# 2noise/ChatTTS

Measured on AMD Instinct MI355X. Metric: audio seconds/sec (RTF), batch=64 per GPU, higher is better.
Workload: dtype f32x3

## Files before the change

### chattts_amd/_lib.py

```python
from __future__ import annotations

import ctypes as C
import os

import numpy as np

import torch

HERE = os.path.dirname(os.path.abspath(__file__))
LIB_PATH = os.environ.get("CTTS_LIB") or os.path.join(HERE, "csrc", "libchattts_amd.so")

F32, BF16 = 0, 1
P = C.c_void_p
PP = C.POINTER(C.c_void_p)


class GptWeights(C.Structure):
    _fields_ = [
        ("n_layers", C.c_int32), ("weight_dtype", C.c_int32), ("kv_dtype", C.c_int32), ("max_pos", C.c_int32),
        ("wqkv", PP), ("wo", PP), ("wgu", PP), ("wd", PP), ("ln1", PP), ("ln2", PP),
        ("norm", P), ("emb_code", P), ("heads", P), ("rope_cos", P), ("rope_sin", P),
        ("rms_eps", C.c_float),
        ("emb_text", P), ("head_text", P), ("n_text", C.c_int32),
        ("wqkv_pk", PP), ("wo_pk", PP), ("wgu_pk", PP), ("wd_pk", PP),
# ... 84 lines not shown
        ("encoder", TrunkWeights), ("decoder", TrunkWeights),
        ("ds0_w", P), ("ds0_b", P), ("ds1_w", P), ("ds1_b", P), ("out_conv_w", P), ("coef", P),
        ("q_in_w", P), ("q_in_b", P), ("q_out_w", P), ("q_out_b", P),
        ("levels", C.c_int32 * 4), ("G", C.c_int32), ("R", C.c_int32), ("D", C.c_int32), ("bound_first", C.c_int32),
        ("mel_window", P), ("mel_fb", P), ("twiddle", P),
    ]


I32, F, SZ = C.c_int32, C.c_float, C.c_size_t

SIGNATURES = {
    "ctts_last_error": (C.c_char_p, []),
    "ctts_version": (C.c_int, []),
    "ctts_gpt_create": (C.c_int, [PP, C.POINTER(GptWeights)]),
    "ctts_gpt_destroy": (None, [P]),
    "ctts_gpt_workspace_bytes": (SZ, [I32, I32]),
    "ctts_gpt_prefill": (C.c_int, [P, C.POINTER(GenState), P, P]),
    "ctts_gpt_prefill_chunk": (C.c_int, [P, C.POINTER(GenState), P, I32, I32, I32, P]),
    "ctts_gpt_decode_step": (C.c_int, [P, C.POINTER(GenState), P]),
    "ctts_gpt_graph_build": (C.c_int, [P, C.POINTER(GenState), P]),
    "ctts_gpt_graph_launch": (C.c_int, [P, I32, P]),
    "ctts_gpt_graph_build_rows": (C.c_int, [P, C.POINTER(GenState), I32, P]),
    "ctts_gpt_graph_launch_rows": (C.c_int, [P, I32, I32, P]),
    "ctts_gpt_graph_destroy": (None, [P]),
    "ctts_gpt_profile_begin": (C.c_int, [P, I32, I32, I32]),
    "ctts_gpt_profile_samples": (C.c_int, [P, C.POINTER(C.c_float), I32, C.POINTER(I32)]),
    "ctts_gpt_profile_end": (C.c_int, [P, C.POINTER(I32), C.POINTER(C.c_double)]),
    "ctts_codec_create": (C.c_int, [PP, C.POINTER(CodecWeights)]),
    "ctts_codec_destroy": (None, [P]),
    "ctts_codec_workspace_bytes": (SZ, [I32, I32]),
# ... 35 lines not shown
    "ctts_dvae_encode_workspace_bytes": (SZ, [I32]),
    "ctts_dvae_decode_workspace_bytes": (SZ, [I32, I32]),
    "ctts_dvae_encode": (C.c_int, [P, P, I32, P, P, SZ, P]),
    "ctts_dvae_decode_codes": (C.c_int, [P, P, P, I32, I32, P, SZ, P]),
    "ctts_k_gemm": (C.c_int, [I32, P, P, P, I32, I32, I32, I32, I32, I32, I32, P, F, P, I32, P, P, I32, I32, I32, I32, I32, P]),
    "ctts_k_gemm_x3p": (C.c_int, [P, P, I32, I32, I32, I32, P, P, P, P, P, P]),
    "ctts_k_gemm_h1p": (C.c_int, [P, P, I32, I32, I32, I32, P, P, P, P, P, P]),
    "ctts_stream_create_cu_mask": (C.c_int, [I32, I32, I32, I32, P]),
    "ctts_stream_destroy": (C.c_int, [P]),
    "ctts_k_mlp_fused": (C.c_int, [P, P, P, I32, I32, P, P, P, P, I32, P]),
    "ctts_k_gemm_fast": (C.c_int, [P, I32, P, I32, I32, I32, P, F, I32, P, I32, P, I32, P, P]),
    "ctts_k_qkv_rope": (C.c_int, [P, P, I32, P, F, P, P, P, I32, P, P, I32, P, P, I32, P]),
    "ctts_k_gemm_dec": (C.c_int, [P, P, I32, I32, I32, P, P, F, I32, P, I32, P, I32, P, I32, P]),
    "ctts_k_gemm_dec32x": (C.c_int, [P, C.c_int64, P, C.c_int64, I32, I32, I32, P, P, I32, F, I32, P, I32, P, I32, P, C.c_int64, I32, P, I32, P, P, P]),
    "ctts_k_gemm_pre_x3": (C.c_int, [P, I32, P, P, I32, I32, I32, I32, I32, P, P, P, I32, P]),
    "ctts_k_dec32_last_variant": (C.c_char_p, []),
    "ctts_k_gemm_dec32": (C.c_int, [P, P, I32, I32, I32, P, P, I32, P, F, I32, P, I32, P, I32, P, I32, I32, I32, P]),
    "ctts_k_rows_prep": (C.c_int, [P, P, P, I32, P]),
    "ctts_k_rope_append": (C.c_int, [P, P, P, I32, I32, P, P, I32, P, P, I32, P]),
    "ctts_k_attention": (C.c_int, [P, P, P, I32, I32, P, I32, P, P, I32, P]),
    "ctts_k_attention_prefill": (C.c_int, [P, P, P, I32, P, I32, I32, P, I32, P]),
    "ctts_k_attention_dec": (C.c_int, [P, P, P, I32, P, P, P, I32, P, P, I32, P]),
    "ctts_k_attention_dec2": (C.c_int, [P, P, P, I32, I32, P, P, P, I32, I32, P]),
    "ctts_k_attention_cfg": (C.c_int, [I32, I32, I32]),
    "ctts_k_attention_heads_per_wg": (C.c_int, [I32]),
    "ctts_rccl_unique_id": (C.c_int, [P]),
    "ctts_rccl_comm_create": (C.c_int, [P, I32, P, I32]),
    "ctts_rccl_comm_destroy": (None, [P]),
    "ctts_broadcast_weights": (C.c_int, [P, P, I32, P, I32, P]),
    "ctts_k_attention_oproj": (C.c_int, [P, P, P, I32, P, P, P, I32, P, P, P, P, P, P]),
# ... 57 lines not shown
```

### chattts_amd/csrc/capi.hip

```cpp
#include <hip/hip_runtime.h>
#include <dlfcn.h>
#include <stdarg.h>
#include <stdio.h>
#include <stdlib.h>
#include <string.h>
#include <algorithm>
#include <map>
#include <vector>

#include "../../include/chattts_amd.h"
#include "kernels.hpp"

static thread_local char g_err[512] = "";
int ctts_fail(const char* fmt, ...) {
  va_list ap;
  va_start(ap, fmt);
  vsnprintf(g_err, sizeof(g_err), fmt, ap);
  va_end(ap);
  return -1;
}
#define fail ctts_fail
#define CK(expr)                                                                                   \
  do {                                                                                             \
    hipError_t _e = (expr);                                                                        \
// ... 11 lines not shown
  std::vector<const void*> wqkv_pk, wo_pk, wgu_pk, wd_pk;
  std::vector<const void*> wo_hd;
  std::vector<const void*> wqkv_x3, wo_x3, wgu_x3, wd_x3;
  bool dec_x3 = false;
  bool qkv_att = false;
  bool att_oproj = false;
  bool dec_packed = false;
  bool dec_packed32 = false;
  bool heads_packed = false;
  int pf_mask = 0;
  int temporal_layers = 0;
  bool pre32_packed = true;
  bool embed_fold = false;
  bool pre_compact = true;
  bool pre_x3 = true;
  bool fnorm_fuse = true;
  std::vector<const float*> ln1, ln2;
  hipGraph_t graph = nullptr;
  hipGraphExec_t exec = nullptr;
  hipGraph_t graph_multi = nullptr;
  hipGraphExec_t exec_multi = nullptr;
  struct RowsGraph { hipGraph_t graph = nullptr, gm = nullptr; hipGraphExec_t exec = nullptr, exec_multi = nullptr; };
  std::map<int, RowsGraph> rows_graphs;
  int multi_steps = 1;
  int prof_tag = -1;
  int prof_max = 0;
  bool skip_finished = true;
  int n_cu = 0;
  int prof_stride = 1;
  int prof_seen = 0;
// ... 92 lines not shown
    g->dec_x3 = true;
  }
  if (w->wo_hd && g->dec_packed) {
    g->wo_hd.assign(w->wo_hd, w->wo_hd + L);
    const char* e = getenv("CTTS_ATT_OPROJ");
    g->att_oproj = e && atoi(e) == 1;
  }
  { const char* e = getenv("CTTS_SKIP_FINISHED"); if (e && atoi(e) == 0) g->skip_finished = false; }
  { const char* e = getenv("CTTS_FNORM_FUSE"); if (e && atoi(e) == 0) g->fnorm_fuse = false; }
  { const char* e = getenv("CTTS_W_TEMPORAL_LAYERS"); if (e) g->temporal_layers = atoi(e); }
  { const char* e = getenv("CTTS_PF"); if (e) g->pf_mask = atoi(e); }
  { const char* e = getenv("CTTS_QKV_ATT"); g->qkv_att = e && atoi(e) == 1; }
  { const char* e = getenv("CTTS_PRE32_PACKED"); if (e && atoi(e) == 0) g->pre32_packed = false; }
  { const char* e = getenv("CTTS_PRE_X3"); if (e && atoi(e) == 0) g->pre_x3 = false; }
  { const char* e = getenv("CTTS_PRE_COMPACT"); if (e && atoi(e) == 0) g->pre_compact = false; }
  { const char* e = getenv("CTTS_EMBED_FOLD"); if (e) g->embed_fold = atoi(e) != 0; }
  {
    int dev = 0, cus = 0;
    const char* e = getenv("CTTS_ATT_SPLIT");
    if (e && atoi(e) == 1 && hipGetDevice(&dev) == hipSuccess &&
        hipDeviceGetAttribute(&cus, hipDeviceAttributeMultiprocessorCount, dev) == hipSuccess && cus > 0 && cus <= ATT_CUS_MAX)
      g->n_cu = cus;
  }
  *out = g;
  return 0;
}

extern "C" void ctts_gpt_graph_destroy(ctts_gpt* g) {
  if (!g) return;
  if (g->exec) { (void)hipGraphExecDestroy(g->exec); g->exec = nullptr; }
  if (g->graph) { (void)hipGraphDestroy(g->graph); g->graph = nullptr; }
  if (g->exec_multi) { (void)hipGraphExecDestroy(g->exec_multi); g->exec_multi = nullptr; }
  if (g->graph_multi) { (void)hipGraphDestroy(g->graph_multi); g->graph_multi = nullptr; }
  for (auto& kv : g->rows_graphs) {
    if (kv.second.exec) (void)hipGraphExecDestroy(kv.second.exec);
    if (kv.second.graph) (void)hipGraphDestroy(kv.second.graph);
    if (kv.second.exec_multi) (void)hipGraphExecDestroy(kv.second.exec_multi);
    if (kv.second.gm) (void)hipGraphDestroy(kv.second.gm);
  }
// ... 254 lines not shown
    d.res = nullptr; d.Cp = ws.actp32; d.kch_out = INTER / 16;
    CK(launch_gemm_pre32(d, ws.rstd, st));
    d.Ap = ws.actp32; d.Wp = (const float*)g->wd_pk[l]; d.N = HID; d.K = INTER; d.norm_w = nullptr; d.epi = EPI_RES;
    d.C = ws.x; d.ldc = HID; d.res = ws.x; d.ldr = HID; d.Cp = ws.xp32; d.kch_out = HID / 16;
    CK(launch_gemm_pre32(d, nullptr, st));
  }
  for (int l = 0; !fast && !packed32 && !pre32 && !x3 && l < g->w.n_layers; ++l) {
    void* kc = (char*)s->kcache + kv_layer * l;
    void* vc = (char*)s->vcache + kv_layer * l;
    GemmArgs a;
    memset(&a, 0, sizeof(a));
    a.taps = 1;
    a.n_active = nact;
    a.A = ws.x; a.lda = HID; a.W = g->wqkv[l]; a.C = ws.qkv; a.ldc = 3 * HID; a.M = M; a.N = 3 * HID; a.K = HID; a.wt = wt;
    a.epi = EPI_STORE; a.norm_w = g->ln1[l]; a.eps = g->w.rms_eps;
    if (pre_x3) { CK(launch_rows_rstd32(ws.x, HID, M, g->w.rms_eps, ws.rstd, st)); CK(launch_gemm_pre_x3(a, ws.rstd, st)); }
    else { Prof p(g, 1, st, prof_ok); CK(launch_gemm_skinny(a, st)); }
    { Prof p(g, 2, st, prof_ok); CK(launch_rope_append(ws.qkv, kc, vc, kt, cmax, g->w.rope_cos, g->w.rope_sin, rm, M, st)); }
    { Prof p(g, 3, st, prof_ok); CK(launch_attention(ws.qkv, kc, vc, kt, cmax, ws.ao, 0, rm, M, st)); }
    a.A = ws.ao; a.lda = HID; a.W = g->wo[l]; a.C = ws.x; a.ldc = HID; a.N = HID; a.K = HID; a.epi = EPI_RES; a.norm_w = nullptr;
    a.res = ws.x; a.ldr = HID;
    if (pre_x3) CK(launch_gemm_pre_x3(a, nullptr, st));
    else { Prof p(g, 4, st, prof_ok); CK(launch_gemm_skinny(a, st)); }
    a.A = ws.x; a.W = g->wgu[l]; a.C = ws.act; a.ldc = INTER; a.N = INTER; a.K = HID; a.epi = EPI_SILU_MUL; a.norm_w = g->ln2[l];
    a.res = nullptr;
    if (pre_x3) { CK(launch_rows_rstd32(ws.x, HID, M, g->w.rms_eps, ws.rstd, st)); CK(launch_gemm_pre_x3(a, ws.rstd, st)); }
    else { Prof p(g, 5, st, prof_ok); CK(launch_gemm_skinny(a, st)); }
    a.A = ws.act; a.lda = INTER; a.W = g->wd[l]; a.C = ws.x; a.ldc = HID; a.N = HID; a.K = INTER; a.epi = EPI_RES; a.norm_w = nullptr;
    a.res = ws.x; a.ldr = HID;
    if (pre_x3) CK(launch_gemm_pre_x3(a, nullptr, st));
    else { Prof p(g, 6, st, prof_ok); CK(launch_gemm_skinny(a, st)); }
  }
  if (!heads) return 0;
  if (fuse_fnorm) {
    const int nlog = s->infer_text ? g->w.n_text : NVQ * NAUDIO;
    Dec32Args d;
    memset(&d, 0, sizeof(d));
    d.Ap = x3 ? ws.hfinp : ws.xp32; d.Wp = s->infer_text ? g->w.head_text_pk : g->w.heads_pk; d.M = Bh; d.N = (nlog + 15) / 16 * 16; d.K = HID; d.n_active = nact;
    d.epi = EPI_STORE; d.C = ws.logits; d.ldc = nlog; d.n_cols = nlog;
    d.fnorm = 1; d.norm_w = g->w.norm; d.eps = g->w.rms_eps; d.desc = ws.desc; d.hid = s->hiddens; d.hid_cap = s->hid_cap ? s->hid_cap : s->max_new;
    d.T = s->T; d.prompt_len = s->prompt_len;
    Prof p(g, 8, st, prof_ok);
    CK(launch_gemm_dec32(d, st));
  } else {
  { Prof p(g, 7, st, prof_ok);
// ... 1176 lines not shown
}
extern "C" int ctts_k_final_norm(const float* x, int32_t q_per_b, const float* w, float eps, float* hfin, float* hiddens,
                                 int32_t max_new, const int32_t* len, int32_t T, int32_t B, void* stream) {
  CK(launch_final_norm(x, q_per_b, w, eps, hfin, hiddens, max_new, len, T, B, nullptr, nullptr, nullptr, (hipStream_t)stream));
  return 0;
}
extern "C" int ctts_k_gemm_pre_x3(const float* A, int32_t lda, const float* W, float* C, int32_t ldc, int32_t M, int32_t N, int32_t K, int32_t epi,
                                  const float* norm_w, const float* rstd, const float* res, int32_t ldr, void* stream) {
  GemmArgs a;
  memset(&a, 0, sizeof(a));
  a.taps = 1; a.A = A; a.lda = lda; a.W = W; a.C = C; a.ldc = ldc; a.M = M; a.N = N; a.K = K; a.wt = WT_F32; a.epi = epi;
  a.norm_w = norm_w; a.res = res; a.ldr = ldr;
  CK(launch_gemm_pre_x3(a, rstd, (hipStream_t)stream));
  return 0;
}
extern "C" int ctts_k_sample(const ctts_gen_state* s, const float* logits, void* stream) {
  if (!s || !logits) return fail("ctts_k_sample: bad arguments");
  CK(launch_sample(make_sample_args(s, logits), (hipStream_t)stream));
  return 0;
}
extern "C" int ctts_k_sample_text(const ctts_gen_state* s, const float* logits, int32_t n_text, void* stream) {
  if (!s || !logits || n_text <= 0 || n_text > NTEXT_MAX) return fail("ctts_k_sample_text: bad arguments");
  CK(launch_sample_text(make_sample_args(s, logits), n_text, (hipStream_t)stream));
  return 0;
}
extern "C" int ctts_k_device_guard_probe(void* stream, int32_t* before, int32_t* stream_dev, int32_t* inside, int32_t* switched) {
  if (!before || !stream_dev || !inside || !switched) return fail("ctts_k_device_guard_probe: null argument");
  int b = -1, in = -1;
  CK(hipGetDevice(&b));
  *stream_dev = -1;
// ... 389 lines not shown
```

### chattts_amd/csrc/kernels.hpp

```cpp
#pragma once
#include <hip/hip_runtime.h>
#include <hip/hip_ext.h>
#include <stdint.h>

#include "common.hpp"

extern thread_local hipEvent_t ctts_prof_start, ctts_prof_stop;
#define CTTS_LAUNCH(kern, grid, block, st, ...)                                                                   \
  do {                                                                                                            \
    if (ctts_prof_start) {                                                                                        \
      hipExtLaunchKernelGGL(kern, grid, block, 0, st, ctts_prof_start, ctts_prof_stop, 0, __VA_ARGS__);           \
      ctts_prof_start = nullptr; ctts_prof_stop = nullptr;                                                        \
    } else {                                                                                                      \
      hipLaunchKernelGGL(kern, grid, block, 0, st, __VA_ARGS__);                                                  \
    }                                                                                                             \
  } while (0)

#define CTTS_LAUNCH_SMEM(kern, grid, block, smem, st, ...)                                                        \
  do {                                                                                                            \
    if (ctts_prof_start) {                                                                                        \
      hipExtLaunchKernelGGL(kern, grid, block, smem, st, ctts_prof_start, ctts_prof_stop, 0, __VA_ARGS__);        \
      ctts_prof_start = nullptr; ctts_prof_stop = nullptr;                                                        \
    } else {                                                                                                      \
      hipLaunchKernelGGL(kern, grid, block, smem, st, __VA_ARGS__);                                               \
// ... 30 lines not shown
  int wt;
  int epi;
  const float* norm_w;
  float eps;
  const float* res; int ldr;
  const float* bias;
  const float* gamma;
  const int32_t* n_active;
  int taps, cin, frames, pad, dil;
  long long* dbg;
  const int2* seg;
};

hipError_t launch_gemm_skinny(const GemmArgs& a, hipStream_t st);
hipError_t launch_gemm_pre_x3(const GemmArgs& a, const float* rstd, hipStream_t st);

enum FastEpi { FEPI_STORE32 = 0, FEPI_RES = 1, FEPI_SILU = 2, FEPI_QKV_ROPE = 3 };
#define SSQ_PARTS 48
struct FastGemmArgs {
  const uint16_t* A; int lda;
  const uint16_t* W;
  int M, N, K;
  const float* ssq_in;
  float eps;
  int epi;
  float* C32; int ldc;
  uint16_t* Cb; int ldcb;
  float* ssq_out;
  int q_per_b; const int32_t* len; const int32_t* kv_start;
  const int32_t* row_map;
// ... 383 lines not shown
```

### chattts_amd/csrc/prefill32x.hip

```cpp
#include <stdlib.h>

#include "common.hpp"
#include "kernels.hpp"

namespace {

constexpr int XBK = 32, XLD = XBK + 8;
constexpr int XNT = 256;

typedef float xf2 __attribute__((ext_vector_type(2)));
typedef _Float16 xb2 __attribute__((ext_vector_type(2)));

__device__ __forceinline__ void split2(const float a, const float b, uint32_t& hi, uint32_t& lo) {
  const xf2 v = {a > 65504.0f ? 65504.0f : (a < -65504.0f ? -65504.0f : a), b > 65504.0f ? 65504.0f : (b < -65504.0f ? -65504.0f : b)};
  const xb2 h = __builtin_convertvector(v, xb2);
  hi = __builtin_bit_cast(uint32_t, h);
  const xf2 hf = __builtin_convertvector(h, xf2);
  const xb2 l = __builtin_convertvector((v - hf) * X3_LO_SCALE, xb2);
  lo = __builtin_bit_cast(uint32_t, l);
}
__device__ __forceinline__ void split4(const float4 v, ushort4& hi, ushort4& lo) {
  uint32_t h0, l0, h1, l1;
  split2(v.x, v.y, h0, l0);
  split2(v.z, v.w, h1, l1);
// ... 116 lines not shown
        const int col = n0 + wn * 32 + cl;
        a.C[(size_t)row * a.ldc + col] = silu_f(acc[i][0][r] * rs) * (acc[i][1][r] * rs);
      } else {
#pragma unroll
        for (int j = 0; j < 2; ++j) {
          const int col = n0 + wn * 64 + j * 32 + cl;
          if (col >= N) continue;
          const float v = acc[i][j][r] * rs;
          a.C[(size_t)row * a.ldc + col] = (EPI == EPI_RES) ? a.res[(size_t)row * a.ldr + col] + v : v;
        }
      }
    }
  }
}

}

hipError_t launch_gemm_pre_x3(const GemmArgs& a, const float* rstd, hipStream_t st) {
  if (a.M <= 0 || a.N <= 0 || a.K <= 0 || (a.K % XBK) || (a.lda & 3) || !a.A || !a.W || !a.C || a.wt != WT_F32 || a.taps != 1) return hipErrorInvalidValue;
  if ((a.norm_w != nullptr) != (rstd != nullptr)) return hipErrorInvalidValue;
  if (a.epi == EPI_SILU_MUL ? (a.N % 64) != 0 : (a.N % 128) != 0) return hipErrorInvalidValue;
  if (a.epi == EPI_RES && !a.res) return hipErrorInvalidValue;
  const dim3 block(XNT);
  const int nx = a.epi == EPI_SILU_MUL ? a.N / 64 : a.N / 128;
  static int force_small = -1;
  if (force_small < 0) { const char* e = getenv("CTTS_PREX3_SMALL"); force_small = e ? atoi(e) : 0; }
  const bool small = force_small == 1 || (force_small != 2 && (long)nx * ((a.M + 127) / 128) < 1024);
  const dim3 grid(nx, small ? (a.M + 63) / 64 : (a.M + 127) / 128);
  switch (a.epi) {
    case EPI_SILU_MUL:
      if (small) CTTS_LAUNCH((gemm_pre_x3_k<EPI_SILU_MUL, 1>), grid, block, st, a, rstd); else CTTS_LAUNCH((gemm_pre_x3_k<EPI_SILU_MUL, 2>), grid, block, st, a, rstd);
      break;
    case EPI_RES:
      if (small) CTTS_LAUNCH((gemm_pre_x3_k<EPI_RES, 1>), grid, block, st, a, rstd); else CTTS_LAUNCH((gemm_pre_x3_k<EPI_RES, 2>), grid, block, st, a, rstd);
      break;
    case EPI_STORE:
      if (small) CTTS_LAUNCH((gemm_pre_x3_k<EPI_STORE, 1>), grid, block, st, a, rstd); else CTTS_LAUNCH((gemm_pre_x3_k<EPI_STORE, 2>), grid, block, st, a, rstd);
      break;
    default: return hipErrorInvalidValue;
  }
  return hipGetLastError();
}
```

### chattts_amd/engine.py

```python
from __future__ import annotations

import ctypes as C
import os
import logging
import math
from dataclasses import dataclass, field
from typing import Iterator, List, Optional, Sequence

import numpy as np
import torch

from . import _lib
from . import flac as FLAC
from . import g711 as G711
from . import loudness as LN
from . import resample as RS
from . import timescale as TS
from ._sync import wait_event, wait_stream
from .config import DVAE, GPT, VOCOS
from .rng import ExpDraws, penalty_table
from .weights import fold_weight_norm, gpt_layer_count

log = logging.getLogger("chattts_amd")

# ... 141 lines not shown


X3_LO_SCALE = 2048.0


def split_f16(w: torch.Tensor):
    w = w.to(torch.float32).clamp(-65504.0, 65504.0)
    hi = w.to(torch.float16)
    lo = ((w - hi.to(torch.float32)) * X3_LO_SCALE).to(torch.float16)
    return hi, lo


def pack_frag_x3(w: torch.Tensor) -> torch.Tensor:
    hi, lo = split_f16(w)
    return torch.stack([pack_frag(hi), pack_frag(lo)], 0).contiguous()


def unpack_frag_x3(p: torch.Tensor, R: int, Cc: int) -> torch.Tensor:
    return unpack_frag(p[0].float(), R, Cc) + unpack_frag(p[1].float(), R, Cc) / X3_LO_SCALE


def pack_wo_heads(wo: torch.Tensor) -> torch.Tensor:
    assert tuple(wo.shape) == (GPT.hidden, GPT.hidden)
    return wo.view(GPT.hidden, GPT.n_heads, 8, 8).permute(1, 2, 0, 3).contiguous()


def pack_frag32(w: torch.Tensor) -> torch.Tensor:
    R, Cc = w.shape
    assert R % 16 == 0 and Cc % 16 == 0
    return w.reshape(R // 16, 16, Cc // 16, 4, 4).permute(0, 2, 3, 1, 4).contiguous()
# ... 93 lines not shown
        w = _lib.GptWeights()
        w.n_layers, w.weight_dtype, w.kv_dtype, w.max_pos = self.n_layers, self.code, self.code, max_pos
        w.wqkv, w.wo, w.wgu, w.wd, w.ln1, w.ln2 = [C.cast(a, _lib.PP) for a in self._arrs]
        w.norm, w.emb_code, w.heads = self.norm.data_ptr(), self.emb_code.data_ptr(), self.heads.data_ptr()
        w.rope_cos, w.rope_sin = self.rope_cos.data_ptr(), self.rope_sin.data_ptr()
        w.rms_eps = float(rms_eps)
        w.emb_text, w.head_text, w.n_text = self.emb_text.data_ptr(), self.head_text.data_ptr(), GPT.n_text
        if self._pk_arrs is not None:
            w.wqkv_pk, w.wo_pk, w.wgu_pk, w.wd_pk = [C.cast(a, _lib.PP) for a in self._pk_arrs]
        w.heads_pk, w.head_text_pk = _lib.ptr(self.heads_pk), _lib.ptr(self.head_text_pk)
        if self._wo_hd_arr is not None:
            w.wo_hd = C.cast(self._wo_hd_arr, _lib.PP)
        if self._x3_arrs is not None:
            w.wqkv_x3, w.wo_x3, w.wgu_x3, w.wd_x3 = [C.cast(a, _lib.PP) for a in self._x3_arrs]
        self._w = w
        h = C.c_void_p()
        _lib.check(self.lib.ctts_gpt_create(C.byref(h), C.byref(w)), "ctts_gpt_create")
        self.handle = h
        spec = codec_cu_spec() if os.environ.get("CTTS_GPT_COMPLEMENT") == "1" else None
        self.stream = cu_masked_stream(self.lib, dev, *spec, True) if spec else torch.cuda.Stream(device=dev)
        self._lane_res = [(self.handle, self.stream)]
        self._lane_res_alt = []
        self._lane_res_text = []
        self.default_lanes = 1
        self.rng = "host"
        self.last_stats = {}
        self._session = None
        self._session_alt = None
        self._session_text = None
        self._draws_cache = None

    def __del__(self):
        try:
            for h, _ in [*getattr(self, "_lane_res", []), *getattr(self, "_lane_res_alt", []), *getattr(self, "_lane_res_text", [])]:
                self.lib.ctts_gpt_destroy(h)
            self._lane_res, self._lane_res_alt, self._lane_res_text = [], [], []
            self.handle = None
        except Exception:
            pass

    def weight_bytes_per_step(self) -> int:
        es = 2 if self.dtype == "bf16" else 4
        per_layer = (3 * 768 * 768 + 768 * 768 + 2 * 3072 * 768 + 768 * 3072) * es
        return per_layer * self.n_layers + self.heads.numel() * 4

    def embed_prompt(self, input_ids: torch.Tensor, text_mask: torch.Tensor) -> torch.Tensor:
        ids = input_ids.to(self.device)
        tm = text_mask.to(self.device).bool()
        et = self.emb_text[ids[..., 0].clamp(0, GPT.n_text - 1)]
        cid = ids.clamp(0, GPT.n_audio - 1)
        ec = self.emb_code[0][cid[..., 0]]
        for k in range(1, GPT.n_vq):
            ec = ec + self.emb_code[k][cid[..., k]]
        return torch.where(tm[..., None], et, ec).contiguous()

    def _lane_resources(self, n: int, pool: str = ""):
        pool = getattr(self, "_lane_res" + pool)
        while len(pool) < n:
            h = C.c_void_p()
            _lib.check(self.lib.ctts_gpt_create(C.byref(h), C.byref(self._w)), "ctts_gpt_create")
            pool.append((h, torch.cuda.Stream(device=self.device)))
        return pool[:n]

    def generate(self, emb: torch.Tensor, inputs_ids: torch.Tensor, temperature: torch.Tensor, eos_token: int = GPT.n_audio - 1,
                 attention_mask: Optional[torch.Tensor] = None, max_new_token: int = 2048, min_new_token: int = 0,
                 logits_processors: Sequence = (), infer_text: bool = False, return_attn: bool = False,
                 return_hidden: bool = False, stream: bool = False, show_tqdm: bool = False, ensure_non_empty: bool = True,
                 stream_batch: int = 24, manual_seed: Optional[int] = None, context: Optional[Context] = None,
                 *, use_graph: bool = True, stop_at: Optional[torch.Tensor] = None, row_offset: int = 0,
                 total_rows: Optional[int] = None, profile_tag: Optional[int] = None,
                 profile_stride: int = 1, lanes: Optional[int] = None,
                 teacher_ids: Optional[torch.Tensor] = None, prefill_chunk: Optional[int] = None,
                 return_sampled: bool = False, rng: Optional[str] = None, rng_seed: Optional[int] = None,
                 rng_nonce=None, row_ids: Optional[torch.Tensor] = None, exact: bool = False,
                 text_rng: Optional[str] = None) -> Iterator[GenerationOutputs]:
        if return_attn:
# ... 1886 lines not shown
```

### chattts_amd/serving.py

```python
from __future__ import annotations

import copy
import ctypes as C
import dataclasses
import itertools
import queue
import threading
import time
from collections import deque
from concurrent.futures import Future
from dataclasses import dataclass, field
from typing import Deque, Iterator, List, Optional, Tuple

import numpy as np
import torch

from . import _lib
from . import flac as FLAC
from . import g711 as G711
from . import loudness as LN
from . import resample as RS
from . import timescale as TS
from ._sync import wait_event, wait_stream
from .config import GPT
# ... 147 lines not shown
        self.nrow = 1 if self.infer_text else GPT.n_vq
        self.V = GPT.n_text if self.infer_text else GPT.n_audio
        if manual_seed is None and rng != "device" and not self.per_request:
            raise NotImplementedError("SlotPool with the host generator needs manual_seed (one constant Exp(1) draw per session); "
                                      "use rng='device' for unseeded sampling")
        if cap > engine.max_pos:
            raise ValueError("slot capacity exceeds max_position_embeddings")
        self.eng, self.S, self.cap, self.hid_cap = engine, slots, cap, hid_cap
        self.lib = engine.lib
        dev = self.dev = engine.device
        if self.infer_text:
            plan = plan_from_processors(())
        else:
            warpers, procs = gen_logits(GPT.n_audio - 1, top_P, top_K, repetition_penalty)
            plan = plan_from_processors((*procs, *warpers))
        h = C.c_void_p()
        _lib.check(self.lib.ctts_gpt_create(C.byref(h), C.byref(engine._w)), "ctts_gpt_create")
        self.handle = h
        self.st = torch.cuda.Stream(device=dev)
        nvq = GPT.n_vq
        with torch.cuda.stream(self.st):
            self.ids_buf = torch.zeros((slots, cap, nvq), dtype=torch.int64, device=dev)
            self.len = torch.ones((slots,), dtype=torch.int32, device=dev)
            self.kv_start = torch.zeros((slots,), dtype=torch.int32, device=dev)
            self._Sp = (slots + 15) // 16 * 16
            self.state_blk = torch.zeros((5 * self._Sp,), dtype=torch.uint8, device=dev)
            self.finish = self.state_blk[:slots]
            self.finish.fill_(1)
            self.end_idx = self.state_blk[self._Sp:].view(torch.int32)[:slots]
            self.prompt_len = torch.ones((slots,), dtype=torch.int32, device=dev)
            self.stop_at = torch.full((slots,), -1, dtype=torch.int32, device=dev)
            self.hiddens = torch.empty((slots, hid_cap, GPT.hidden), dtype=torch.float32, device=dev)
            kv_shape = (engine.n_layers, slots, GPT.n_heads, cap, GPT.head_dim)
# ... 939 lines not shown
```

### include/chattts_amd.h

```cpp
#ifndef CHATTTS_AMD_H
#define CHATTTS_AMD_H

#include <stddef.h>
#include <stdint.h>

#ifdef __cplusplus
extern "C" {
#endif

#define CTTS_F32 0
#define CTTS_BF16 1

typedef struct ctts_gpt ctts_gpt;
typedef struct ctts_codec ctts_codec;

const char* ctts_last_error(void);
int ctts_version(void);

typedef struct {
  int32_t n_layers;
  int32_t weight_dtype;
  int32_t kv_dtype;
  int32_t max_pos;
  const void* const* wqkv;
// ... 75 lines not shown
  int64_t* sampled_ids;
  const int32_t* order;
  int32_t rng_device;
  int32_t rng_per_step;
  const uint64_t* rng_seed;
  const uint32_t* rng_nonce;
  float* margin;
  const int32_t* row_base;
  int32_t proj_exact;
  int32_t prefill_valid_rows;
  const ctts_sampling_row* row_sampling;
} ctts_gen_state;

int ctts_gpt_create(ctts_gpt** out, const ctts_gpt_weights* w);
void ctts_gpt_destroy(ctts_gpt* g);
size_t ctts_gpt_workspace_bytes(int32_t B, int32_t T);

int ctts_gpt_prefill(ctts_gpt* g, const ctts_gen_state* s, const float* emb, void* stream);
int ctts_gpt_prefill_chunk(ctts_gpt* g, const ctts_gen_state* s, const float* emb_chunk, int32_t t0, int32_t tc, int32_t last, void* stream);
int ctts_gpt_decode_step(ctts_gpt* g, const ctts_gen_state* s, void* stream);
int ctts_gpt_graph_build(ctts_gpt* g, const ctts_gen_state* s, void* stream);
int ctts_gpt_graph_launch(ctts_gpt* g, int32_t n_steps, void* stream);
int ctts_gpt_graph_build_rows(ctts_gpt* g, const ctts_gen_state* s, int32_t rows, void* stream);
int ctts_gpt_graph_launch_rows(ctts_gpt* g, int32_t n_steps, int32_t rows, void* stream);
void ctts_gpt_graph_destroy(ctts_gpt* g);

int ctts_gpt_profile_begin(ctts_gpt* g, int32_t tag, int32_t max_samples, int32_t stride );
int ctts_gpt_profile_samples(ctts_gpt* g, float* ms_out, int32_t cap, int32_t* n_samples);
int ctts_gpt_profile_end(ctts_gpt* g, int32_t* n_samples, double* total_ms);

// ... 239 lines not shown
                    uint16_t* vcache, int32_t cmax, const float* cos_tab, const float* sin_tab, int32_t q_per_b, const int32_t* len,
                    const int32_t* kv_start, int32_t force_mb, void* stream);
int ctts_k_gemm_dec(const uint16_t* Ap, const uint16_t* Wp, int32_t M, int32_t N, int32_t K, const int32_t* n_active, const float* ssq_in,
                    float eps, int32_t epi, float* C32, int32_t ldc, uint16_t* Cp, int32_t kch_out, float* ssq_out, int32_t force_mb,
                    void* stream);
int ctts_k_gemm_dec32(const float* Ap, const float* Wp, int32_t M, int32_t N, int32_t K, const int32_t* n_active, const float* X, int32_t ldx,
                      const float* norm_w, float eps, int32_t epi, float* C, int32_t ldc, const float* res, int32_t ldr, float* Cp,
                      int32_t kch_out, int32_t force_mb, int32_t n_cols ,
                      void* stream);
int ctts_k_gemm_dec32x(const uint16_t* Ap, int64_t a_plane, const uint16_t* Wp, int64_t w_plane, int32_t M, int32_t N, int32_t K,
                       const int32_t* n_active, const float* X, int32_t ldx, float eps, int32_t epi, float* C, int32_t ldc, const float* res,
                       int32_t ldr, uint16_t* Cp, int64_t c_plane, int32_t kch_out, float* Cp32, int32_t force_mb, const float* ssq_in,
                       float* ssq_out, void* stream);
int ctts_k_gemm_pre_x3(const float* A, int32_t lda, const float* W, float* C, int32_t ldc, int32_t M, int32_t N, int32_t K, int32_t epi,
                       const float* norm_w, const float* rstd, const float* res, int32_t ldr, void* stream);
const char* ctts_k_dec32_last_variant(void);
int ctts_k_rows_prep(const float* x32, uint16_t* xb, float* ssq, int32_t M, void* stream);
int ctts_k_rope_append(float* qkv, void* kcache, void* vcache, int32_t kv_dtype, int32_t cmax, const float* cos_tab, const float* sin_tab,
                       int32_t q_per_b, const int32_t* len, const int32_t* kv_start, int32_t M, void* stream);
int ctts_k_attention(const float* qkv, const void* kcache, const void* vcache, int32_t kv_dtype, int32_t cmax, float* out,
                     int32_t q_per_b, const int32_t* len, const int32_t* kv_start, int32_t M, void* stream);
int ctts_k_attention_prefill(const float* qkv, const uint16_t* kcache, const uint16_t* vcache, int32_t cmax, float* out, int32_t q_per_b,
                             int32_t slot0, const int32_t* kv_start, int32_t M, void* stream);
int ctts_k_attention_dec(const float* qkv, const uint16_t* kcache, const uint16_t* vcache, int32_t cmax, uint16_t* out_packed,
                         const int32_t* desc, const int32_t* n_active, int32_t M, float* part, int32_t* cnt, int32_t n_cu, void* stream);
int ctts_k_attention_dec2(const float* qkv, const void* kcache, const void* vcache, int32_t kv_dtype, int32_t cmax, void* out_packed,
                          const int32_t* desc, const int32_t* n_active, int32_t covers_all, int32_t M, void* stream);
int ctts_k_attention_cfg(int32_t persist, int32_t workgroups, int32_t ring);
int ctts_k_attention_heads_per_wg(int32_t hpw);
int ctts_k_attention_oproj(const float* qkv, const uint16_t* kcache, const uint16_t* vcache, int32_t cmax, const uint16_t* wo_hd,
// ... 40 lines not shown
```

Before: 1117.

## Add prefill x3 GEMM using pre-split f16 weight planes in MFMA fragment layout

Weights for the four prefill GEMMs per layer are pre-split into hi/lo f16 planes and packed in MFMA fragment order at load time. A new kernel streams them into LDS with global_load_lds in a three-slot ring, and runs the three-pass f16 emulation of f32. This removes the per-tile f32-to-f16 split of weights inside the prefill GEMM. The cost is extra device memory for the packed planes, plus a new path that is on by default for f32x3 and can be turned off with an env var.

```diff
diff --git a/chattts_amd/_lib.py b/chattts_amd/_lib.py
--- a/chattts_amd/_lib.py
+++ b/chattts_amd/_lib.py
@@ -122,6 +122,7 @@
     "ctts_version": (C.c_int, []),
     "ctts_gpt_create": (C.c_int, [PP, C.POINTER(GptWeights)]),
     "ctts_gpt_destroy": (None, [P]),
+    "ctts_gpt_set_prefill_planes": (C.c_int, [P, I32, I32, P]),
     "ctts_gpt_workspace_bytes": (SZ, [I32, I32]),
     "ctts_gpt_prefill": (C.c_int, [P, C.POINTER(GenState), P, P]),
     "ctts_gpt_prefill_chunk": (C.c_int, [P, C.POINTER(GenState), P, I32, I32, I32, P]),
@@ -187,6 +188,7 @@
     "ctts_k_gemm_dec": (C.c_int, [P, P, I32, I32, I32, P, P, F, I32, P, I32, P, I32, P, I32, P]),
     "ctts_k_gemm_dec32x": (C.c_int, [P, C.c_int64, P, C.c_int64, I32, I32, I32, P, P, I32, F, I32, P, I32, P, I32, P, C.c_int64, I32, P, I32, P, P, P]),
     "ctts_k_gemm_pre_x3": (C.c_int, [P, I32, P, P, I32, I32, I32, I32, I32, P, P, P, I32, P]),
+    "ctts_k_gemm_pre_x3p": (C.c_int, [P, I32, P, P, I32, I32, I32, I32, I32, P, P, P, I32, P]),
     "ctts_k_dec32_last_variant": (C.c_char_p, []),
     "ctts_k_gemm_dec32": (C.c_int, [P, P, I32, I32, I32, P, P, I32, P, F, I32, P, I32, P, I32, P, I32, I32, I32, P]),
     "ctts_k_rows_prep": (C.c_int, [P, P, P, I32, P]),
diff --git a/chattts_amd/csrc/capi.hip b/chattts_amd/csrc/capi.hip
--- a/chattts_amd/csrc/capi.hip
+++ b/chattts_amd/csrc/capi.hip
@@ -49,6 +49,8 @@
   bool embed_fold = false;
   bool pre_compact = true;
   bool pre_x3 = true;
+  std::vector<const uint16_t*> pre_planes[4];
+  bool pre_x3_planes = true;
   bool fnorm_fuse = true;
   std::vector<const float*> ln1, ln2;
   hipGraph_t graph = nullptr;
@@ -171,6 +173,8 @@
   { const char* e = getenv("CTTS_PRE32_PACKED"); if (e && atoi(e) == 0) g->pre32_packed = false; }
   { const char* e = getenv("CTTS_PRE_X3"); if (e && atoi(e) == 0) g->pre_x3 = false; }
   { const char* e = getenv("CTTS_PRE_COMPACT"); if (e && atoi(e) == 0) g->pre_compact = false; }
+  { const char* e = getenv("CTTS_PRE_X3_PLANES"); if (e && atoi(e) == 0) g->pre_x3_planes = false; }
+  for (auto& v : g->pre_planes) v.assign(L, nullptr);
   { const char* e = getenv("CTTS_EMBED_FOLD"); if (e) g->embed_fold = atoi(e) != 0; }
   {
     int dev = 0, cus = 0;
@@ -180,6 +184,13 @@
       g->n_cu = cus;
   }
   *out = g;
+  return 0;
+}
+
+extern "C" int ctts_gpt_set_prefill_planes(ctts_gpt* g, int32_t layer, int32_t which, const uint16_t* planes) {
+  if (!g || layer < 0 || layer >= g->w.n_layers || which < 0 || which > 3) return fail("ctts_gpt_set_prefill_planes: bad arguments");
+  if ((reinterpret_cast<uintptr_t>(planes) & 15) != 0) return fail("ctts_gpt_set_prefill_planes: planes must be 16-byte aligned");
+  g->pre_planes[which][layer] = planes;
   return 0;
 }
 
@@ -464,21 +475,23 @@
     a.n_active = nact;
     a.A = ws.x; a.lda = HID; a.W = g->wqkv[l]; a.C = ws.qkv; a.ldc = 3 * HID; a.M = M; a.N = 3 * HID; a.K = HID; a.wt = wt;
     a.epi = EPI_STORE; a.norm_w = g->ln1[l]; a.eps = g->w.rms_eps;
-    if (pre_x3) { CK(launch_rows_rstd32(ws.x, HID, M, g->w.rms_eps, ws.rstd, st)); CK(launch_gemm_pre_x3(a, ws.rstd, st)); }
+    const bool planes = pre_x3 && g->pre_x3_planes && g->pre_planes[0][l] && g->pre_planes[1][l] && g->pre_planes[2][l] && g->pre_planes[3][l];
+    auto pre_gemm = [&](int which, const float* rstd) { return planes ? launch_gemm_pre_x3p(a, rstd, g->pre_planes[which][l], st) : launch_gemm_pre_x3(a, rstd, st); };
+    if (pre_x3) { CK(launch_rows_rstd32(ws.x, HID, M, g->w.rms_eps, ws.rstd, st)); CK(pre_gemm(0, ws.rstd)); }
     else { Prof p(g, 1, st, prof_ok); CK(launch_gemm_skinny(a, st)); }
     { Prof p(g, 2, st, prof_ok); CK(launch_rope_append(ws.qkv, kc, vc, kt, cmax, g->w.rope_cos, g->w.rope_sin, rm, M, st)); }
     { Prof p(g, 3, st, prof_ok); CK(launch_attention(ws.qkv, kc, vc, kt, cmax, ws.ao, 0, rm, M, st)); }
     a.A = ws.ao; a.lda = HID; a.W = g->wo[l]; a.C = ws.x; a.ldc = HID; a.N = HID; a.K = HID; a.epi = EPI_RES; a.norm_w = nullptr;
     a.res = ws.x; a.ldr = HID;
-    if (pre_x3) CK(launch_gemm_pre_x3(a, nullptr, st));
+    if (pre_x3) CK(pre_gemm(1, nullptr));
     else { Prof p(g, 4, st, prof_ok); CK(launch_gemm_skinny(a, st)); }
     a.A = ws.x; a.W = g->wgu[l]; a.C = ws.act; a.ldc = INTER; a.N = INTER; a.K = HID; a.epi = EPI_SILU_MUL; a.norm_w = g->ln2[l];
     a.res = nullptr;
-    if (pre_x3) { CK(launch_rows_rstd32(ws.x, HID, M, g->w.rms_eps, ws.rstd, st)); CK(launch_gemm_pre_x3(a, ws.rstd, st)); }
+    if (pre_x3) { CK(launch_rows_rstd32(ws.x, HID, M, g->w.rms_eps, ws.rstd, st)); CK(pre_gemm(2, ws.rstd)); }
     else { Prof p(g, 5, st, prof_ok); CK(launch_gemm_skinny(a, st)); }
     a.A = ws.act; a.lda = INTER; a.W = g->wd[l]; a.C = ws.x; a.ldc = HID; a.N = HID; a.K = INTER; a.epi = EPI_RES; a.norm_w = nullptr;
     a.res = ws.x; a.ldr = HID;
-    if (pre_x3) CK(launch_gemm_pre_x3(a, nullptr, st));
+    if (pre_x3) CK(pre_gemm(3, nullptr));
     else { Prof p(g, 6, st, prof_ok); CK(launch_gemm_skinny(a, st)); }
   }
   if (!heads) return 0;
@@ -1685,6 +1698,15 @@
   CK(launch_gemm_pre_x3(a, rstd, (hipStream_t)stream));
   return 0;
 }
+extern "C" int ctts_k_gemm_pre_x3p(const float* A, int32_t lda, const uint16_t* Wp, float* C, int32_t ldc, int32_t M, int32_t N, int32_t K, int32_t epi,
+                                   const float* norm_w, const float* rstd, const float* res, int32_t ldr, void* stream) {
+  GemmArgs a;
+  memset(&a, 0, sizeof(a));
+  a.taps = 1; a.A = A; a.lda = lda; a.W = nullptr; a.C = C; a.ldc = ldc; a.M = M; a.N = N; a.K = K; a.wt = WT_F32; a.epi = epi;
+  a.norm_w = norm_w; a.res = res; a.ldr = ldr;
+  CK(launch_gemm_pre_x3p(a, rstd, Wp, (hipStream_t)stream));
+  return 0;
+}
 extern "C" int ctts_k_sample(const ctts_gen_state* s, const float* logits, void* stream) {
   if (!s || !logits) return fail("ctts_k_sample: bad arguments");
   CK(launch_sample(make_sample_args(s, logits), (hipStream_t)stream));
diff --git a/chattts_amd/csrc/kernels.hpp b/chattts_amd/csrc/kernels.hpp
--- a/chattts_amd/csrc/kernels.hpp
+++ b/chattts_amd/csrc/kernels.hpp
@@ -68,6 +68,7 @@
 
 hipError_t launch_gemm_skinny(const GemmArgs& a, hipStream_t st);
 hipError_t launch_gemm_pre_x3(const GemmArgs& a, const float* rstd, hipStream_t st);
+hipError_t launch_gemm_pre_x3p(const GemmArgs& a, const float* rstd, const uint16_t* Wp, hipStream_t st);
 
 enum FastEpi { FEPI_STORE32 = 0, FEPI_RES = 1, FEPI_SILU = 2, FEPI_QKV_ROPE = 3 };
 #define SSQ_PARTS 48
diff --git a/chattts_amd/csrc/prefill32x.hip b/chattts_amd/csrc/prefill32x.hip
--- a/chattts_amd/csrc/prefill32x.hip
+++ b/chattts_amd/csrc/prefill32x.hip
@@ -154,6 +154,143 @@
   }
 }
 
+constexpr int PFRAG = 512;
+constexpr int PSLOT = 16 * PFRAG;
+constexpr int PNSLOT = 3;
+
+#define XP_GLL(g, l) __builtin_amdgcn_global_load_lds((const __attribute__((address_space(1))) void*)(g), (__attribute__((address_space(3))) void*)(l), 16, 0, 0)
+
+template <int EPI>
+__global__ __launch_bounds__(XNT, 2) void gemm_pre_x3p_k(GemmArgs a, const float* __restrict__ rstd, const uint16_t* __restrict__ Wp) {
+  constexpr bool SILU = EPI == EPI_SILU_MUL;
+  constexpr int BM = 64;
+  constexpr int BNO = SILU ? 64 : 128;
+  constexpr int ABUF = 8 * PFRAG;
+  __shared__ __attribute__((aligned(16))) uint16_t lds[PNSLOT * PSLOT + 2 * ABUF + 2 * BM];
+  uint16_t* const Wr = lds;
+  uint16_t* const As = lds + PNSLOT * PSLOT;
+  float* const rstd_s = reinterpret_cast<float*>(lds + PNSLOT * PSLOT + 2 * ABUF);
+
+  const int tid = threadIdx.x, wave = tid >> 6, lane = tid & 63;
+  const int wm = wave & 1, wn = wave >> 1;
+  const int M = a.M, N = a.N, K = a.K;
+  const int m0 = blockIdx.y * BM, n0 = blockIdx.x * BNO;
+  const int kb16 = K >> 4, nk = K / XBK;
+
+  if (rstd != nullptr && tid < BM) rstd_s[tid] = rstd[min(m0 + tid, M - 1)];
+
+  const uint16_t* wg = Wp + ((size_t)(blockIdx.x * 4 + wave) * kb16) * 2 * PFRAG + lane * 8;
+  auto issue_w = [&](int s) {
+    uint16_t* lw = Wr + (s % PNSLOT) * PSLOT + wave * 4 * PFRAG;
+    const uint16_t* g = wg + (size_t)s * 4 * PFRAG;
+#pragma unroll
+    for (int p = 0; p < 4; ++p) XP_GLL(g + p * PFRAG, lw + p * PFRAG);
+  };
+
+  const int lr = tid >> 3, lq = tid & 7, lk = lq * 4;
+  const float* ap[2];
+#pragma unroll
+  for (int p = 0; p < 2; ++p) ap[p] = a.A + (size_t)min(m0 + lr + 32 * p, M - 1) * a.lda + lk;
+  const int aw_off = ((lq >> 2) * 2) * PFRAG + ((((lq >> 1) & 1) << 5) + (lr ^ ((lq >> 1) << 1))) * 8 + (lq & 1) * 4;
+  float4 ra[2], rg;
+#define XP_FETCH(K0)                                                                                              \
+  do {                                                                                                            \
+    _Pragma("unroll") for (int p = 0; p < 2; ++p) ra[p] = *reinterpret_cast<const float4*>(ap[p] + (K0));          \
+    rg = a.norm_w != nullptr ? *reinterpret_cast<const float4*>(a.norm_w + (K0) + lk) : make_float4(1.f, 1.f, 1.f, 1.f); \
+  } while (0)
+#define XP_STAGE(SB)                                                                                              \
+  do {                                                                                                            \
+    _Pragma("unroll") for (int p = 0; p < 2; ++p) {                                                               \
+      ushort4 h, l;                                                                                               \
+      split4(make_float4(ra[p].x * rg.x, ra[p].y * rg.y, ra[p].z * rg.z, ra[p].w * rg.w), h, l);                  \
+      *reinterpret_cast<ushort4*>(As + (SB) * ABUF + p * 4 * PFRAG + aw_off) = h;                                 \
+      *reinterpret_cast<ushort4*>(As + (SB) * ABUF + p * 4 * PFRAG + aw_off + PFRAG) = l;                         \
+    }                                                                                                             \
+  } while (0)
+
+  f32x16 acc[2], accx[2];
+#pragma unroll
+  for (int j = 0; j < 2; ++j)
+#pragma unroll
+    for (int r = 0; r < 16; ++r) { acc[j][r] = 0.f; accx[j][r] = 0.f; }
+
+  issue_w(0);
+  if (nk > 1) issue_w(1);
+  asm volatile("" ::: "memory");
+  XP_FETCH(0);
+  XP_STAGE(0);
+  if (nk > 1) XP_FETCH(XBK);
+
+  const int hl = lane >> 5, ri = lane & 31;
+  const int ar_off0 = wm * 4 * PFRAG + ((hl << 5) + (ri ^ (hl << 1))) * 8;
+  const int ar_off1 = wm * 4 * PFRAG + 2 * PFRAG + ((hl << 5) + (ri ^ ((2 + hl) << 1))) * 8;
+  const int wt0 = SILU ? wn : wn * 2, wt1 = SILU ? 2 + wn : wn * 2 + 1;
+  for (int s = 0; s < nk; ++s) {
+    if (s + 1 < nk) asm volatile("s_waitcnt vmcnt(7)" ::: "memory"); else asm volatile("s_waitcnt vmcnt(0)" ::: "memory");
+    asm volatile("s_waitcnt lgkmcnt(0)" ::: "memory");
+    __builtin_amdgcn_s_barrier();
+    asm volatile("" ::: "memory");
+    if (s + 1 < nk) XP_STAGE((s + 1) & 1);
+    const uint16_t* la = As + (s & 1) * ABUF;
+    const uint16_t* lw = Wr + (s % PNSLOT) * PSLOT + lane * 8;
+    f16x8 wh0[2], wl0[2], wh1[2], wl1[2], ah[2], al[2];
+#pragma unroll
+    for (int kb = 0; kb < 2; ++kb) {
+      wh0[kb] = *reinterpret_cast<const f16x8*>(lw + ((wt0 * 2 + kb) * 2 + 0) * PFRAG);
+      wl0[kb] = *reinterpret_cast<const f16x8*>(lw + ((wt0 * 2 + kb) * 2 + 1) * PFRAG);
+      wh1[kb] = *reinterpret_cast<const f16x8*>(lw + ((wt1 * 2 + kb) * 2 + 0) * PFRAG);
+      wl1[kb] = *reinterpret_cast<const f16x8*>(lw + ((wt1 * 2 + kb) * 2 + 1) * PFRAG);
+      ah[kb] = *reinterpret_cast<const f16x8*>(la + (kb ? ar_off1 : ar_off0));
+      al[kb] = *reinterpret_cast<const f16x8*>(la + (kb ? ar_off1 : ar_off0) + PFRAG);
+    }
+    asm volatile("" ::: "memory");
+    if (s + 2 < nk) {
+      XP_FETCH((s + 2) * XBK);
+      asm volatile("" ::: "memory");
+      issue_w(s + 2);
+    }
+#pragma unroll
+    for (int kb = 0; kb < 2; ++kb) {
+      f32x16 x0 = accx[0], x1 = accx[1];
+      x0 = __builtin_amdgcn_mfma_f32_32x32x16_f16(al[kb], wh0[kb], x0, 0, 0, 0);
+      x1 = __builtin_amdgcn_mfma_f32_32x32x16_f16(al[kb], wh1[kb], x1, 0, 0, 0);
+      x0 = __builtin_amdgcn_mfma_f32_32x32x16_f16(ah[kb], wl0[kb], x0, 0, 0, 0);
+      x1 = __builtin_amdgcn_mfma_f32_32x32x16_f16(ah[kb], wl1[kb], x1, 0, 0, 0);
+      accx[0] = x0; accx[1] = x1;
+      acc[0] = __builtin_amdgcn_mfma_f32_32x32x16_f16(ah[kb], wh0[kb], acc[0], 0, 0, 0);
+      acc[1] = __builtin_amdgcn_mfma_f32_32x32x16_f16(ah[kb], wh1[kb], acc[1], 0, 0, 0);
+    }
+  }
+#undef XP_FETCH
+#undef XP_STAGE
+
+#pragma unroll
+  for (int j = 0; j < 2; ++j)
+#pragma unroll
+    for (int r = 0; r < 16; ++r) acc[j][r] += accx[j][r] * X3_LO_INV;
+  const int cl = lane & 31;
+#pragma unroll
+  for (int r = 0; r < 16; ++r) {
+    const int lrow = wm * 32 + (r & 3) + 8 * (r >> 2) + 4 * (lane >> 5);
+    const int row = m0 + lrow;
+    if (row >= M) continue;
+    const float rs = rstd != nullptr ? rstd_s[lrow] : 1.0f;
+    if (EPI == EPI_SILU_MUL) {
+      const int col = n0 + wn * 32 + cl;
+      a.C[(size_t)row * a.ldc + col] = silu_f(acc[0][r] * rs) * (acc[1][r] * rs);
+    } else {
+#pragma unroll
+      for (int j = 0; j < 2; ++j) {
+        const int col = n0 + wn * 64 + j * 32 + cl;
+        if (col >= N) continue;
+        const float v = acc[j][r] * rs;
+        a.C[(size_t)row * a.ldc + col] = (EPI == EPI_RES) ? a.res[(size_t)row * a.ldr + col] + v : v;
+      }
+    }
+  }
+}
+#undef XP_GLL
+
 }
 
 hipError_t launch_gemm_pre_x3(const GemmArgs& a, const float* rstd, hipStream_t st) {
@@ -181,3 +318,19 @@
   }
   return hipGetLastError();
 }
+
+hipError_t launch_gemm_pre_x3p(const GemmArgs& a, const float* rstd, const uint16_t* Wp, hipStream_t st) {
+  if (a.M <= 0 || a.N <= 0 || a.K <= 0 || (a.K % XBK) || (a.lda & 3) || !a.A || !Wp || !a.C || a.taps != 1) return hipErrorInvalidValue;
+  if ((reinterpret_cast<uintptr_t>(Wp) & 15) != 0) return hipErrorInvalidValue;
+  if ((a.norm_w != nullptr) != (rstd != nullptr)) return hipErrorInvalidValue;
+  if (a.epi == EPI_SILU_MUL ? (a.N % 64) != 0 : (a.N % 128) != 0) return hipErrorInvalidValue;
+  if (a.epi == EPI_RES && !a.res) return hipErrorInvalidValue;
+  const dim3 block(XNT), grid(a.epi == EPI_SILU_MUL ? a.N / 64 : a.N / 128, (a.M + 63) / 64);
+  switch (a.epi) {
+    case EPI_SILU_MUL: CTTS_LAUNCH((gemm_pre_x3p_k<EPI_SILU_MUL>), grid, block, st, a, rstd, Wp); break;
+    case EPI_RES: CTTS_LAUNCH((gemm_pre_x3p_k<EPI_RES>), grid, block, st, a, rstd, Wp); break;
+    case EPI_STORE: CTTS_LAUNCH((gemm_pre_x3p_k<EPI_STORE>), grid, block, st, a, rstd, Wp); break;
+    default: return hipErrorInvalidValue;
+  }
+  return hipGetLastError();
+}
diff --git a/chattts_amd/engine.py b/chattts_amd/engine.py
--- a/chattts_amd/engine.py
+++ b/chattts_amd/engine.py
@@ -179,6 +179,23 @@
 def pack_frag_x3(w: torch.Tensor) -> torch.Tensor:
     hi, lo = split_f16(w)
     return torch.stack([pack_frag(hi), pack_frag(lo)], 0).contiguous()
+
+
+def prefill_row_order(R: int, paired: bool) -> torch.Tensor:
+    if not paired:
+        return torch.arange(R)
+    n = R // 2
+    assert R % 2 == 0 and n % 64 == 0
+    t = torch.arange(n // 64)[:, None, None] * 64 + torch.arange(64)[None, None, :]
+    return (t + torch.tensor([0, n])[None, :, None]).reshape(-1)
+
+
+def pack_prefill_planes(w: torch.Tensor, paired: bool = False) -> torch.Tensor:
+    R, K = w.shape
+    assert R % 128 == 0 and K % 32 == 0
+    hi, lo = split_f16(w[prefill_row_order(R, paired).to(w.device)])
+    frag = lambda t: t.reshape(R // 32, 32, K // 16, 2, 8).permute(0, 2, 3, 1, 4).reshape(R // 32, K // 16, 64, 8)
+    return torch.stack([frag(hi), frag(lo)], 2).contiguous()
 
 
 def unpack_frag_x3(p: torch.Tensor, R: int, Cc: int) -> torch.Tensor:
@@ -302,9 +319,10 @@
         if self._x3_arrs is not None:
             w.wqkv_x3, w.wo_x3, w.wgu_x3, w.wd_x3 = [C.cast(a, _lib.PP) for a in self._x3_arrs]
         self._w = w
-        h = C.c_void_p()
-        _lib.check(self.lib.ctts_gpt_create(C.byref(h), C.byref(w)), "ctts_gpt_create")
-        self.handle = h
+        self.pre_planes = None
+        if dtype == "f32x3" and os.environ.get("CTTS_PRE_X3_PLANES", "1") != "0" and os.environ.get("CTTS_PRE_X3", "1") != "0":
+            self.pre_planes = [[pack_prefill_planes(t, paired=(k == 2)) for t in ws] for k, ws in enumerate((self.wqkv, self.wo, self.wgu, self.wd))]
+        self.handle = self.new_handle()
         spec = codec_cu_spec() if os.environ.get("CTTS_GPT_COMPLEMENT") == "1" else None
         self.stream = cu_masked_stream(self.lib, dev, *spec, True) if spec else torch.cuda.Stream(device=dev)
         self._lane_res = [(self.handle, self.stream)]
@@ -318,6 +336,15 @@
         self._session_text = None
         self._draws_cache = None
 
+    def new_handle(self) -> C.c_void_p:
+        h = C.c_void_p()
+        _lib.check(self.lib.ctts_gpt_create(C.byref(h), C.byref(self._w)), "ctts_gpt_create")
+        if self.pre_planes is not None:
+            for k, ws in enumerate(self.pre_planes):
+                for l, t in enumerate(ws):
+                    _lib.check(self.lib.ctts_gpt_set_prefill_planes(h, l, k, t.data_ptr()), "ctts_gpt_set_prefill_planes")
+        return h
+
     def __del__(self):
         try:
             for h, _ in [*getattr(self, "_lane_res", []), *getattr(self, "_lane_res_alt", []), *getattr(self, "_lane_res_text", [])]:
@@ -345,9 +372,7 @@
     def _lane_resources(self, n: int, pool: str = ""):
         pool = getattr(self, "_lane_res" + pool)
         while len(pool) < n:
-            h = C.c_void_p()
-            _lib.check(self.lib.ctts_gpt_create(C.byref(h), C.byref(self._w)), "ctts_gpt_create")
-            pool.append((h, torch.cuda.Stream(device=self.device)))
+            pool.append((self.new_handle(), torch.cuda.Stream(device=self.device)))
         return pool[:n]
 
     def generate(self, emb: torch.Tensor, inputs_ids: torch.Tensor, temperature: torch.Tensor, eos_token: int = GPT.n_audio - 1,
diff --git a/chattts_amd/serving.py b/chattts_amd/serving.py
--- a/chattts_amd/serving.py
+++ b/chattts_amd/serving.py
@@ -185,9 +185,7 @@
         else:
             warpers, procs = gen_logits(GPT.n_audio - 1, top_P, top_K, repetition_penalty)
             plan = plan_from_processors((*procs, *warpers))
-        h = C.c_void_p()
-        _lib.check(self.lib.ctts_gpt_create(C.byref(h), C.byref(engine._w)), "ctts_gpt_create")
-        self.handle = h
+        self.handle = engine.new_handle()
         self.st = torch.cuda.Stream(device=dev)
         nvq = GPT.n_vq
         with torch.cuda.stream(self.st):
diff --git a/include/chattts_amd.h b/include/chattts_amd.h
--- a/include/chattts_amd.h
+++ b/include/chattts_amd.h
@@ -113,6 +113,7 @@
 
 int ctts_gpt_create(ctts_gpt** out, const ctts_gpt_weights* w);
 void ctts_gpt_destroy(ctts_gpt* g);
+int ctts_gpt_set_prefill_planes(ctts_gpt* g, int32_t layer, int32_t which, const uint16_t* planes);
 size_t ctts_gpt_workspace_bytes(int32_t B, int32_t T);
 
 int ctts_gpt_prefill(ctts_gpt* g, const ctts_gen_state* s, const float* emb, void* stream);
@@ -382,6 +383,8 @@
                        float* ssq_out, void* stream);
 int ctts_k_gemm_pre_x3(const float* A, int32_t lda, const float* W, float* C, int32_t ldc, int32_t M, int32_t N, int32_t K, int32_t epi,
                        const float* norm_w, const float* rstd, const float* res, int32_t ldr, void* stream);
+int ctts_k_gemm_pre_x3p(const float* A, int32_t lda, const uint16_t* Wp, float* C, int32_t ldc, int32_t M, int32_t N, int32_t K, int32_t epi,
+                        const float* norm_w, const float* rstd, const float* res, int32_t ldr, void* stream);
 const char* ctts_k_dec32_last_variant(void);
 int ctts_k_rows_prep(const float* x32, uint16_t* xb, float* ssq, int32_t M, void* stream);
 int ctts_k_rope_append(float* qkv, void* kcache, void* vcache, int32_t kv_dtype, int32_t cmax, const float* cos_tab, const float* sin_tab,
```

Result: no change. 1108 (-0.7%).
